# iammadab/zk

Measured on AMD Instinct MI355X. Metric: field-ops/sec (MLE fold, 2^24 evals, BN254 Fr) + sumcheck prover wall-clock, higher is better.
Workload: dtype u256 (8 x u32 Montgomery limbs, integer)

## Files before the change

zk_amd/csrc/common.cuh:

```cuda
#pragma once
#include "field.cuh"

namespace zk {

constexpr int kBlock = 256;
constexpr int kMaxFactors = 8;

struct FactorPtrs {
    const uint64_t *in[kMaxFactors];
    uint64_t *out[kMaxFactors];
};

constexpr int kMaxBatch = 8;
template <class Slot>
struct BatchOf {
    Slot a[kMaxBatch];
};
struct FactorPtrs4 {
    const uint64_t *in[4];
    uint64_t *out[4];
};
ZK_HD FactorPtrs4 factor_ptrs4(const FactorPtrs &f) {
    FactorPtrs4 r;
    for (int i = 0; i < 4; ++i) r.in[i] = f.in[i], r.out[i] = f.out[i];
// ... 95 lines not shown
struct ClaimJob {
    const uint64_t *prev_rp;
    const uint64_t *prev_chal;
    const uint64_t *w;
    uint64_t *out;
    uint32_t ns;
};
ZK_HD Fe lead_rebuild(uint32_t D, const Fe *S, const FieldParams &P) {
    const Fe L = S[D];
    if (D == 1) return fe_add(S[0], L, P);
    if (D == 2) {
        const Fe a = fe_add(S[1], L, P);
        return fe_sub(fe_add(a, a, P), S[0], P);
    }
    Fe b = fe_add(fe_sub(S[2], S[1], P), fe_add(L, L, P), P);
    b = fe_add(fe_add(b, b, P), b, P);
    return fe_add(S[0], b, P);
}

template <int CTRL>
ZK_D Fe fe_dpp(const Fe &s) {
    Fe o;
#pragma unroll
    for (int i = 0; i < 8; ++i) o.v[i] = __builtin_amdgcn_update_dpp(0u, s.v[i], CTRL, 0xF, 0xF, true);
    return o;
}
ZK_D Fe fe_wave_sum(Fe s, const FieldParams &P, uint32_t width = 64) {
    if (width > 32) {
        Fe a, b;
#pragma unroll
        for (int i = 0; i < 8; ++i) {
            const auto r = __builtin_amdgcn_permlane32_swap(s.v[i], s.v[i], false, false);
            a.v[i] = r[0];
            b.v[i] = r[1];
        }
        s = fe_add(a, b, P);
    }
    if (width > 16) {
        Fe a, b;
#pragma unroll
        for (int i = 0; i < 8; ++i) {
            const auto r = __builtin_amdgcn_permlane16_swap(s.v[i], s.v[i], false, false);
            a.v[i] = r[0];
            b.v[i] = r[1];
        }
        s = fe_add(a, b, P);
    }
    if (width > 8) s = fe_add(s, fe_dpp<0x128>(s), P);
    if (width > 4) s = fe_add(s, fe_dpp<0x12C>(s), P);
    if (width > 2) s = fe_add(s, fe_dpp<0x12E>(s), P);
    if (width > 1) s = fe_add(s, fe_dpp<0x12F>(s), P);
    return s;
}
ZK_D Fe claim_eval(const ClaimJob &cj, const FieldParams &P) {
    const uint32_t lane = threadIdx.x & 63;
    const Fe r = fe_load(cj.prev_chal, 0);
    Fe term = fe_zero();
    if (lane < cj.ns) {
        Fe one;
#pragma unroll
        for (int i = 0; i < 8; ++i) one.v[i] = P.r1[i];
        term = fe_mul(fe_load(cj.prev_rp, lane), fe_load(cj.w, lane), P);
        Fe node = fe_zero();
        for (uint32_t u = 0; u < cj.ns; ++u) {
            if (u != lane) term = fe_mul(term, fe_sub(r, node, P), P);
            node = fe_add(node, one, P);
        }
    }
    return fe_wave_sum(term, P, 8);
}

constexpr int kEvalHighMax = 12;
struct EvalHighPoint {
    uint32_t n;
    uint32_t r[kEvalHighMax][8];
};
ZK_D uint32_t eval_high_lane(uint32_t n) { return n > 8 ? 15u : n > 4 ? 7u : n > 2 ? 3u : n > 1 ? 1u : 0u; }
ZK_D Fe eval_high_weight(const EvalHighPoint &ph, uint64_t g, uint32_t lane, const FieldParams &P) {
    Fe one;
#pragma unroll
    for (int i = 0; i < 8; ++i) one.v[i] = P.r1[i];
    Fe f = one;
    for (uint32_t k = 0; k < ph.n; ++k) {
        Fe r;
#pragma unroll
        for (int i = 0; i < 8; ++i) r.v[i] = ph.r[k][i];
        const Fe sel = (g >> k) & 1 ? r : fe_sub(one, r, P);
        if ((lane & 15) == k) f = sel;
    }
    if (ph.n > 8) f = fe_mul(f, fe_dpp<0x128>(f), P);
    if (ph.n > 4) f = fe_mul(f, fe_dpp<0x124>(f), P);
    if (ph.n > 2) f = fe_mul(f, fe_dpp<0x122>(f), P);
    if (ph.n > 1) f = fe_mul(f, fe_dpp<0x121>(f), P);
    return f;
}

ZK_D Fe block_scan_excl(Fe x, Fe *red, const FieldParams &P, Fe *total) {
    const uint32_t t = threadIdx.x;
    red[t] = x;
    __syncthreads();
    for (uint32_t h = 1; h < kBlock; h <<= 1) {
        const Fe y = t >= h ? fe_mul_tt(red[t - h], red[t], P) : red[t];
        __syncthreads();
        red[t] = y;
        __syncthreads();
    }
// ... 9 lines not shown
```

zk_amd/csrc/field.cuh:

```cuda
#pragma once
#include <stdint.h>

#if defined(__HIPCC__)
#include <hip/hip_runtime.h>
#define ZK_HD __host__ __device__ __forceinline__
#define ZK_D __device__ __forceinline__
#else
#define ZK_HD inline
#define ZK_D inline
#endif

namespace zk {

struct FieldParams {
    uint32_t p[8];
    uint32_t r1[8];
    uint32_t r2[8];
    uint32_t inv;
    uint32_t bits;
    uint32_t p29[9];
    uint32_t inv29;
    uint32_t r2_29[9];
    uint32_t r2s_29[9];
};
// ... 305 lines not shown
        }
#pragma unroll
        for (int i = 0; i < 9; ++i) s[i] = borrow ? s[i] : d[i];
    }
}

struct WideAcc {
    uint32_t v[17];
};
ZK_HD void wide_zero(WideAcc &w) {
#pragma unroll
    for (int i = 0; i < 17; ++i) w.v[i] = 0;
}
template <int C>
ZK_HD void wide_mac_col(WideAcc &w, Acc &acc, const uint32_t a[8], const uint32_t b[8]) {
    constexpr int lo = C < 8 ? 0 : C - 7, hi = C < 8 ? C : 7;
    acc_add32(acc, w.v[C]);
    mac_col<hi - lo + 1>(acc, a + lo, b + (C - lo));
    w.v[C] = acc_shift(acc);
    if constexpr (C + 1 < 15) wide_mac_col<C + 1>(w, acc, a, b);
}
ZK_HD void wide_mac(WideAcc &w, const uint32_t a[8], const uint32_t b[8]) {
    Acc acc = {0, 0};
    wide_mac_col<0>(w, acc, a, b);
    acc_add32(acc, w.v[15]);
    w.v[15] = acc_shift(acc);
    w.v[16] += (uint32_t)acc.lh;
}
constexpr int kMaxLazy = 32;
ZK_HD Fe redc_wide(const WideAcc &w, const FieldParams &P) {
    uint32_t m[8];
    Acc acc = {0, 0};
    uint32_t s[9];
    redc_cols<0>(w.v, m, s, acc, P);
    s[8] = (uint32_t)acc.lh;
    {
        uint64_t c = 0;
        const uint32_t top = w.v[16];
#pragma unroll
        for (int i = 0; i < 8; ++i) {
            c += (uint64_t)top * P.r1[i] + s[i];
            s[i] = (uint32_t)c;
            c >>= 32;
        }
        s[8] += (uint32_t)c;
    }
    ladder9<4>(s, P);
    Fe r;
#pragma unroll
    for (int i = 0; i < 8; ++i) r.v[i] = s[i];
    return r;
}

ZK_HD Fe fe_reduce_u256(const uint32_t x[8], const FieldParams &P) {
    uint32_t s[9];
#pragma unroll
    for (int i = 0; i < 8; ++i) s[i] = x[i];
    s[8] = 0;
    ladder9<4>(s, P);
    Fe r;
#pragma unroll
    for (int i = 0; i < 8; ++i) r.v[i] = s[i];
    return r;
}

struct Mul29 {
    uint32_t l[9];
};
ZK_HD void split29(const uint32_t a[8], uint32_t out[9]) {
    constexpr uint32_t M = (1u << 29) - 1;
#pragma unroll
    for (int i = 0; i < 9; ++i) {
        const int bit = 29 * i, w = bit >> 5, sh = bit & 31;
        uint32_t v = a[w] >> sh;
        if (sh > 3 && w + 1 < 8) v |= a[w + 1] << (32 - sh);
        out[i] = (i < 8) ? (v & M) : v;
    }
}
ZK_HD Mul29 mul29_prepare(const Fe &c, const FieldParams &P) {
    Fe t = c;
#pragma unroll
    for (int i = 0; i < 5; ++i) t = fe_add(t, t, P);
    Mul29 m;
    split29(t.v, m.l);
    return m;
}
template <bool LAZY = false, bool TWO = false>
ZK_HD Fe mul29_core(const uint32_t (&x)[9], const uint32_t (&y)[9], const Mul29 &c, const FieldParams &P, const Mul29 *c2 = nullptr) {
    constexpr uint32_t M = (1u << 29) - 1;
    uint32_t m[9], r[9];
    uint64_t acc = 0;
#pragma unroll
    for (int k = 0; k < 9; ++k) {
#pragma unroll
        for (int i = 0; i <= k; ++i) acc += (uint64_t)x[i] * c.l[k - i];
        if constexpr (TWO) {
#pragma unroll
            for (int i = 0; i <= k; ++i) acc += (uint64_t)y[i] * c2->l[k - i];
        }
#pragma unroll
        for (int i = 0; i < k; ++i) acc += (uint64_t)m[i] * P.p29[k - i];
        m[k] = ((uint32_t)acc * P.inv29) & M;
        acc += (uint64_t)m[k] * P.p29[0];
        acc >>= 29;
    }
#pragma unroll
// ... 75 lines not shown
```

zk_amd/csrc/host_field.hpp:

```cpp
#pragma once
#include <stdint.h>
#include <string.h>

#include "field.cuh"

namespace zk {

struct FieldInfo {
    FieldParams P;
    uint32_t two_adicity;
    uint32_t generator;
    Fe two_adic_root;
    bool ready;
};

inline const uint64_t *field_modulus_limbs(int field) {
    static const uint64_t M[3][4] = {
        {0x43e1f593f0000001ULL, 0x2833e84879b97091ULL, 0xb85045b68181585dULL, 0x30644e72e131a029ULL},
        {0xffffffff00000001ULL, 0x53bda402fffe5bfeULL, 0x3339d80809a1d805ULL, 0x73eda753299d7d48ULL},
        {0x0a11800000000001ULL, 0x59aa76fed0000001ULL, 0x60b44d1e5c37b001ULL, 0x12ab655e9a2ca556ULL},
    };
    return (field >= 0 && field < 3) ? M[field] : nullptr;
}

// ... 26 lines not shown
    }
    return acc;
}
inline Fe fe_inverse(const Fe &a, const FieldParams &P) {
    uint32_t e[8], two[8] = {2, 0, 0, 0, 0, 0, 0, 0};
    sub8(e, P.p, two);
    return fe_pow_limbs(a, e, P);
}

inline const FieldInfo *field_info(int field) {
    static FieldInfo info[3];
    static const uint32_t adicity[3] = {28, 32, 47};
    static const uint32_t gen[3] = {5, 7, 22};
    if (field < 0 || field > 2) return nullptr;
    FieldInfo &I = info[field];
    if (I.ready) return &I;
    FieldParams &P = I.P;
    Fe pm = fe_from_u64limbs(field_modulus_limbs(field));
    memcpy(P.p, pm.v, 32);
    uint32_t x = 1;
    for (int i = 0; i < 5; ++i) x *= 2u - P.p[0] * x;
    P.inv = 0u - x;
    int top = 7;
    while (top > 0 && P.p[top] == 0) --top;
    P.bits = 32 * top + (32 - __builtin_clz(P.p[top]));
    uint32_t v[8] = {1, 0, 0, 0, 0, 0, 0, 0}, d[8];
    for (int i = 0; i < 512; ++i) {
        uint32_t c = add8(v, v, v);
        uint32_t b = sub8(d, v, P.p);
        if (c | (b ^ 1u)) memcpy(v, d, 32);
        if (i == 255) memcpy(P.r1, v, 32);
    }
    memcpy(P.r2, v, 32);
    split29(P.p, P.p29);
    P.inv29 = P.inv & ((1u << 29) - 1);
    {
        Fe r2;
        memcpy(r2.v, P.r2, 32);
        const Mul29 k0 = mul29_prepare(r2, P);
        Fe r2s = r2;
        for (int i = 0; i < 5; ++i) r2s = fe_add(r2s, r2s, P);
        const Mul29 k1 = mul29_prepare(r2s, P);
        memcpy(P.r2_29, k0.l, sizeof k0.l);
        memcpy(P.r2s_29, k1.l, sizeof k1.l);
    }
    {
        const int rp_log = 257 - (int)P.bits;
        int lazy_log = 0;
        while ((1 << lazy_log) < kMaxLazy) ++lazy_log;
        const int top_log = lazy_log + 2 * (int)P.bits - 512;
        const uint64_t rp = rp_log >= 0 && rp_log < 32 ? (1ull << rp_log) : ~0ull;
        const uint64_t top = top_log < 0 ? 0 : (top_log < 32 ? (1ull << top_log) : ~0ull);
        if (rp_log < 0 || rp + 1 + top >= 32 || rp + 1 + top < rp) return nullptr;
    }
    I.two_adicity = adicity[field];
    I.generator = gen[field];
    uint32_t t[8], one[8] = {1, 0, 0, 0, 0, 0, 0, 0};
    sub8(t, P.p, one);
    for (uint32_t s = 0; s < I.two_adicity; ++s) {
        for (int i = 0; i < 7; ++i) t[i] = (t[i] >> 1) | (t[i + 1] << 31);
        t[7] >>= 1;
    }
    I.two_adic_root = fe_pow_limbs(fe_from_u32(I.generator, P), t, P);
    I.ready = true;
    return &I;
}

inline bool field_root_of_unity(const FieldInfo &I, uint32_t log_n, Fe &out) {
    if (log_n > I.two_adicity) return false;
    Fe w = I.two_adic_root;
    for (uint32_t i = log_n; i < I.two_adicity; ++i) w = fe_sqr(w, I.P);
    out = w;
    return true;
}

inline void fe_to_bytes_be(const Fe &a, const FieldParams &P, uint8_t out[32]) {
    Fe c = fe_to_canonical(a, P);
    for (int i = 0; i < 8; ++i)
        for (int b = 0; b < 4; ++b) out[31 - (4 * i + b)] = (uint8_t)(c.v[i] >> (8 * b));
}
inline Fe fe_from_be_bytes_mod_order(const uint8_t *bytes, size_t len, const FieldParams &P) {
    Fe acc = fe_zero();
    const Fe c256 = fe_from_u32(256, P);
    for (size_t i = 0; i < len; ++i) acc = fe_add(fe_mul(acc, c256, P), fe_from_u32(bytes[i], P), P);
    return acc;
}

}
```

zk_amd/csrc/round_kernels.cuh:

```cuda
#pragma once
#include "common.cuh"
#include "quad.cuh"

namespace zk {

template <int NS, bool SKIP1 = false>
ZK_D void block_reduce_store(Fe (&sum)[NS], uint64_t *__restrict__ partials, const FieldParams &P) {
    __shared__ uint32_t red[kBlock / 64][NS][8];
    const int lane = threadIdx.x & 63, wave = threadIdx.x >> 6;
#pragma unroll
    for (int t = 0; t < NS; ++t) {
        if (SKIP1 && t == 1) continue;
        sum[t] = fe_wave_sum(sum[t], P);
        if (lane == 0) {
#pragma unroll
            for (int i = 0; i < 8; ++i) red[wave][t][i] = sum[t].v[i];
        }
    }
    __syncthreads();
    if (threadIdx.x < NS && !(SKIP1 && threadIdx.x == 1)) {
        const int t = threadIdx.x;
        Fe acc;
#pragma unroll
        for (int i = 0; i < 8; ++i) acc.v[i] = red[0][t][i];
        for (int w = 1; w < kBlock / 64; ++w) {
            Fe o;
#pragma unroll
            for (int i = 0; i < 8; ++i) o.v[i] = red[w][t][i];
            acc = fe_add(acc, o, P);
        }
        fe_store(partials, (uint64_t)blockIdx.x * NS + t, acc);
    }
}

template <int D, bool FUSED>
__global__ __launch_bounds__(kBlock) void k_round(FactorPtrs fp, int k, uint64_t q, FieldParams P,
                                                  const uint64_t *__restrict__ rptr, uint64_t *__restrict__ partials) {
    constexpr int NS = D + 1;
    Mul29 r = {};
    if (FUSED) r = load_challenge29(rptr);
    Fe sum[NS];
    WideAcc acc[NS];
#pragma unroll
    for (int t = 0; t < NS; ++t) {
        sum[t] = fe_zero();
        wide_zero(acc[t]);
    }
    int lazy = 0;
    const uint64_t stride = (uint64_t)gridDim.x * kBlock;
    for (uint64_t j = (uint64_t)blockIdx.x * kBlock + threadIdx.x; j < q; j += stride) {
        Fe prod[NS];
        for (int f = 0; f < k; ++f) {
            Fe lo, hi;
            if (FUSED) {
                const Fe a0 = fe_load(fp.in[f], j), a1 = fe_load(fp.in[f], j + q);
                const Fe a2 = fe_load(fp.in[f], j + 2 * q), a3 = fe_load(fp.in[f], j + 3 * q);
                lo = fe_sub(a0, fe_mul29(fe_sub(a0, a2, P), r, P), P);
                hi = fe_sub(a1, fe_mul29(fe_sub(a1, a3, P), r, P), P);
                fe_store(fp.out[f], j, lo);
                fe_store(fp.out[f], j + q, hi);
            } else {
                lo = fe_load(fp.in[f], j);
                hi = fe_load(fp.in[f], j + q);
            }
            const Fe diff = fe_sub(hi, lo, P);
            Fe v = lo;
#pragma unroll
            for (int t = 0; t < NS; ++t) {
                if (t == 1) v = hi;
                else if (t > 1) v = fe_add(v, diff, P);
                if (k == 1) sum[t] = fe_add(sum[t], v, P);
                else if (f == 0) prod[t] = v;
                else if (f < k - 1) prod[t] = fe_mul(prod[t], v, P);
                else wide_mac(acc[t], prod[t].v, v.v);
            }
        }
        if (k > 1 && ++lazy == kMaxLazy) {
#pragma unroll
            for (int t = 0; t < NS; ++t) {
                sum[t] = fe_add(sum[t], redc_wide(acc[t], P), P);
                wide_zero(acc[t]);
            }
            lazy = 0;
        }
// ... 72 lines not shown
}
#ifndef ZK_KD_MIN_BLOCKS
#define ZK_KD_MIN_BLOCKS(K, EXTRA, FUSED, SKIP1) (((K) + (EXTRA) <= 2 || ((K) == 3 && (EXTRA) == 0) || ((EXTRA) == 1 && (FUSED) && (SKIP1))) ? 2 : 1)
#endif
template <int K, int D, bool FUSED, int EXTRA = 0, bool SKIP1 = false, bool LEAD = false>
ZK_D void round_kd_body(const FactorPtrs &fp, uint64_t q, const FieldParams &P, const uint64_t *__restrict__ rptr, uint64_t *__restrict__ partials,
                        const ClaimJob &cj) {
    constexpr int NS = D + 1, NL = FUSED ? 4 : 2;
    uint32_t nblk = gridDim.x;
    if constexpr (SKIP1) {
        if (cj.out) {
            nblk -= 1;
            if (blockIdx.x == nblk) {
                if (threadIdx.x < 64) {
                    const Fe claim = claim_eval(cj, P);
                    if (threadIdx.x == 0) fe_store(cj.out, 0, claim);
                }
                return;
            }
        }
    }
    Mul29 r = {};
    if (FUSED) r = load_challenge29(rptr);
    RoundRegs<K, D, FUSED, EXTRA> R;
#pragma unroll
    for (int t = 0; t < NS; ++t) {
        R.sum[t] = fe_zero();
        if (EXTRA) R.sum_b[t] = fe_zero();
        if (K > 1) wide_zero(R.acc[t]);
    }
    const uint64_t stride = (uint64_t)nblk * kBlock;
    uint64_t j = (uint64_t)blockIdx.x * kBlock + threadIdx.x;
    if (j < q) {
#pragma unroll
        for (int f = 0; f < K + EXTRA; ++f)
#pragma unroll
            for (int l = 0; l < NL; ++l) R.cur[f][l] = fe_load(fp.in[f], j + (uint64_t)l * q);
    }
    if (RoundRegs<K, D, FUSED, EXTRA>::DEEP && j + stride < q) {
#pragma unroll
        for (int f = 0; f < K + EXTRA; ++f)
#pragma unroll
            for (int l = 0; l < NL; ++l) R.nxt[f][l] = fe_load(fp.in[f], j + stride + (uint64_t)l * q);
    }
    while (j < q) {
        const uint64_t jn = j + stride, jnn = jn + stride;
        const bool more = jn < q, more2 = jnn < q;
        round_factor<0, K, D, FUSED, EXTRA, SKIP1, LEAD>(R, fp, j, jn, more, q, r, P, jnn, more2);
        if constexpr (K + EXTRA > 1) round_factor<1, K, D, FUSED, EXTRA, SKIP1, LEAD>(R, fp, j, jn, more, q, r, P, jnn, more2);
        if constexpr (K + EXTRA > 2) round_factor<2, K, D, FUSED, EXTRA, SKIP1, LEAD>(R, fp, j, jn, more, q, r, P, jnn, more2);
        if constexpr (K + EXTRA > 3) round_factor<3, K, D, FUSED, EXTRA, SKIP1, LEAD>(R, fp, j, jn, more, q, r, P, jnn, more2);
        j = jn;
    }
    if (K > 1) {
#pragma unroll
        for (int t = 0; t < NS; ++t)
            if (!(SKIP1 && t == 1)) R.sum[t] = redc_wide(R.acc[t], P);
    }
    if (EXTRA) {
#pragma unroll
        for (int t = 0; t < NS; ++t)
            if (!(SKIP1 && t == 1)) R.sum[t] = fe_add(R.sum[t], R.sum_b[t], P);
    }
    block_reduce_store<NS, SKIP1>(R.sum, partials, P);
}
template <int K, int D, bool FUSED, int EXTRA = 0, bool SKIP1 = false, bool LEAD = false>
__global__ __launch_bounds__(kBlock, ZK_KD_MIN_BLOCKS(K, EXTRA, FUSED, SKIP1)) void k_round_kd(FactorPtrs fp, uint64_t q, FieldParams P,
                                                        const uint64_t *__restrict__ rptr, uint64_t *__restrict__ partials, ClaimJob cj = {}) {
    round_kd_body<K, D, FUSED, EXTRA, SKIP1, LEAD>(fp, q, P, rptr, partials, cj);
}
struct RoundSlot {
    FactorPtrs4 fp;
    const uint64_t *rptr;
    uint64_t *partials;
    ClaimJob cj;
};
template <int K, int D, bool FUSED, int EXTRA = 0, bool SKIP1 = false, bool LEAD = false>
__global__ __launch_bounds__(kBlock, ZK_KD_MIN_BLOCKS(K, EXTRA, FUSED, SKIP1)) void k_round_kd_b(BatchOf<RoundSlot> b, uint64_t q, FieldParams P) {
    const RoundSlot &a = b.a[blockIdx.y];
    const FactorPtrs fp = factor_ptrs_of(a.fp);
    round_kd_body<K, D, FUSED, EXTRA, SKIP1, LEAD>(fp, q, P, a.rptr, a.partials, a.cj);
}

ZK_D void dot29_mac(uint64_t (&c)[17], const uint32_t (&x)[9], const uint32_t (&y)[9]) {
#if defined(__HIP_DEVICE_COMPILE__) && !defined(ZK_NO_ASM)
    asm("v_mad_u64_u32 %0, vcc, %13, %18, %0\n\t"
        "v_mad_u64_u32 %1, vcc, %13, %19, %1\n\t"
        "v_mad_u64_u32 %2, vcc, %13, %20, %2\n\t"
        "v_mad_u64_u32 %3, vcc, %13, %21, %3\n\t"
        "v_mad_u64_u32 %4, vcc, %13, %22, %4\n\t"
        "v_mad_u64_u32 %5, vcc, %13, %23, %5\n\t"
        "v_mad_u64_u32 %6, vcc, %13, %24, %6\n\t"
        "v_mad_u64_u32 %7, vcc, %13, %25, %7\n\t"
        "v_mad_u64_u32 %8, vcc, %13, %26, %8\n\t"
        "v_mad_u64_u32 %1, vcc, %14, %18, %1\n\t"
        "v_mad_u64_u32 %2, vcc, %14, %19, %2\n\t"
        "v_mad_u64_u32 %3, vcc, %14, %20, %3\n\t"
        "v_mad_u64_u32 %4, vcc, %14, %21, %4\n\t"
        "v_mad_u64_u32 %5, vcc, %14, %22, %5\n\t"
        "v_mad_u64_u32 %6, vcc, %14, %23, %6\n\t"
        "v_mad_u64_u32 %7, vcc, %14, %24, %7\n\t"
        "v_mad_u64_u32 %8, vcc, %14, %25, %8\n\t"
        "v_mad_u64_u32 %9, vcc, %14, %26, %9\n\t"
        "v_mad_u64_u32 %2, vcc, %15, %18, %2\n\t"
        "v_mad_u64_u32 %3, vcc, %15, %19, %3\n\t"
        "v_mad_u64_u32 %4, vcc, %15, %20, %4\n\t"
        "v_mad_u64_u32 %5, vcc, %15, %21, %5\n\t"
        "v_mad_u64_u32 %6, vcc, %15, %22, %6\n\t"
        "v_mad_u64_u32 %7, vcc, %15, %23, %7\n\t"
        "v_mad_u64_u32 %8, vcc, %15, %24, %8\n\t"
        "v_mad_u64_u32 %9, vcc, %15, %25, %9\n\t"
        "v_mad_u64_u32 %10, vcc, %15, %26, %10\n\t"
        "v_mad_u64_u32 %3, vcc, %16, %18, %3\n\t"
        "v_mad_u64_u32 %4, vcc, %16, %19, %4\n\t"
        "v_mad_u64_u32 %5, vcc, %16, %20, %5\n\t"
        "v_mad_u64_u32 %6, vcc, %16, %21, %6\n\t"
        "v_mad_u64_u32 %7, vcc, %16, %22, %7\n\t"
// ... 101 lines not shown
    const uint64_t stride = (uint64_t)gridDim.x * kBlock;
    uint64_t j = (uint64_t)blockIdx.x * kBlock + threadIdx.x;
    if (j < q) {
#pragma unroll
        for (int f = 0; f < NT; ++f) cur[f][0] = fe_load(fp.in[f], j), cur[f][1] = fe_load(fp.in[f], j + q);
    }
    if (DEEP && j + stride < q) {
#pragma unroll
        for (int f = 0; f < NT; ++f) nxt[f][0] = fe_load(fp.in[f], j + stride), nxt[f][1] = fe_load(fp.in[f], j + stride + q);
    }
    int since = 0;
    while (j < q) {
        const uint64_t jn = j + stride, jnn = jn + stride;
        Fe v[NT][2];
#pragma unroll
        for (int f = 0; f < NT; ++f) v[f][0] = cur[f][0], v[f][1] = cur[f][1];
        if (DEEP) {
#pragma unroll
            for (int f = 0; f < NT; ++f) cur[f][0] = nxt[f][0], cur[f][1] = nxt[f][1];
            if (jnn < q) {
#pragma unroll
                for (int f = 0; f < NT; ++f) nxt[f][0] = fe_load(fp.in[f], jnn), nxt[f][1] = fe_load(fp.in[f], jnn + q);
            }
        } else if (jn < q) {
#pragma unroll
            for (int f = 0; f < NT; ++f) cur[f][0] = fe_load(fp.in[f], jn), cur[f][1] = fe_load(fp.in[f], jn + q);
        }
        uint32_t a[9], b[9];
        split29(v[0][0].v, a);
        split29(v[1][0].v, b);
        dot29_mac(c0, a, b);
        split29(v[0][1].v, a);
        split29(v[1][1].v, b);
        dot29_mac(c1, a, b);
        const Fe d0 = fe_sub(v[0][1], v[0][0], P), d1 = fe_sub(v[1][1], v[1][0], P);
        split29(d0.v, a);
        split29(d1.v, b);
        dot29_mac(cL, a, b);
        if (EXTRA) {
            sb0 = fe_add(sb0, v[NT - 1][0], P);
            sb1 = fe_add(sb1, v[NT - 1][1], P);
        }
        if (++since == 7) {
            dot29_normalise(c0);
            dot29_normalise(c1);
            dot29_normalise(cL);
            since = 0;
        }
        j = jn;
    }
    dot29_normalise(c0);
    dot29_normalise(c1);
    dot29_normalise(cL);
    Fe sum[3];
    {
        WideAcc w;
        dot29_to_wide(c0, w);
        sum[0] = redc_wide(w, P);
        dot29_to_wide(c1, w);
        sum[1] = redc_wide(w, P);
        dot29_to_wide(cL, w);
        sum[2] = redc_wide(w, P);
    }
    if (EXTRA) {
        sum[0] = fe_add(sum[0], sb0, P);
        sum[1] = fe_add(sum[1], sb1, P);
    }
    block_reduce_store<3>(sum, partials, P);
}
template <int EXTRA>
__global__ __launch_bounds__(kBlock, 2) void k_round0_dot29(FactorPtrs fp, uint64_t q, FieldParams P, uint64_t *__restrict__ partials) {
    round0_dot29_body<EXTRA>(fp, q, P, partials);
}
template <int EXTRA>
__global__ __launch_bounds__(kBlock, 2) void k_round0_dot29_b(BatchOf<RoundSlot> b, uint64_t q, FieldParams P) {
    const RoundSlot &a = b.a[blockIdx.y];
    const FactorPtrs fp = factor_ptrs_of(a.fp);
    round0_dot29_body<EXTRA>(fp, q, P, a.partials);
}

extern __shared__ __attribute__((aligned(1024))) uint8_t glds_ring[];
constexpr uint32_t kGldsRingBytes = 4 * 8192, kGldsRing3Bytes = 4 * 12288;
template <int N>
ZK_D void wait_vm() {
    asm volatile("s_waitcnt vmcnt(%0)" ::"n"(N) : "memory");
}
#define ZK_GLDS_PIECES(ADDR)                      \
    "global_load_lds_dwordx4 %1, " ADDR " nt\n\t" \
    "global_load_lds_dwordx4 %1, " ADDR " offset:1024 nt\n\t"
#define ZK_GLDS_ROW(M0, ADDR) "s_mov_b32 m0, " M0 "\n\ts_nop 0\n\t" ZK_GLDS_PIECES(ADDR)
ZK_D void glds_rows2(uint64_t a0, uint64_t a1, uint32_t voff, uint32_t lds_dst) {
    unsigned keep;
    asm volatile("s_mov_b32 %0, m0\n\t" ZK_GLDS_ROW("%4", "%2") ZK_GLDS_ROW("%5", "%3") "s_mov_b32 m0, %0"
                 : "=&s"(keep)
                 : "v"(voff), "s"(a0), "s"(a1), "s"(lds_dst), "s"(lds_dst + 2048u)
                 : "memory");
}
ZK_D void glds_rows4(uint64_t a0, uint64_t a1, uint64_t a2, uint64_t a3, uint32_t voff, uint32_t lds_dst) {
    unsigned keep;
    asm volatile("s_mov_b32 %0, m0\n\t" ZK_GLDS_ROW("%6", "%2") ZK_GLDS_ROW("%7", "%3") ZK_GLDS_ROW("%8", "%4") ZK_GLDS_ROW("%9", "%5") "s_mov_b32 m0, %0"
                 : "=&s"(keep)
                 : "v"(voff), "s"(a0), "s"(a1), "s"(a2), "s"(a3), "s"(lds_dst), "s"(lds_dst + 2048u), "s"(lds_dst + 4096u), "s"(lds_dst + 6144u)
                 : "memory");
}
#undef ZK_GLDS_ROW
#undef ZK_GLDS_PIECES
ZK_D Fe glds_elem(const uint8_t *row, uint32_t elem) {
    const uint4 *p = reinterpret_cast<const uint4 *>(row + elem * 32);
    const uint4 a = p[0], b = p[1];
    Fe r = {{a.x, a.y, a.z, a.w, b.x, b.y, b.z, b.w}};
    return r;
}
struct GldsWave {
    uint8_t *my;
    uint32_t my_lds;
    uint32_t lane, voff, own;
    uint64_t r0, rs, K;
};
ZK_D GldsWave glds_wave(uint64_t q, uint32_t nblk, uint32_t bytes_per_wave = 8192) {
    GldsWave w;
    w.lane = threadIdx.x & 63;
// ... 116 lines not shown
    if (F + 1 < NT) {
        const uint64_t a = (uint64_t)(uintptr_t)fp.in[F + 1 < NT ? F + 1 : 0] + run * 2048;
        glds_rows4(a, a + rowb, a + 2 * rowb, a + 3 * rowb, w.voff, w.my_lds);
    } else if (!last) {
        const uint64_t a = (uint64_t)(uintptr_t)fp.in[0] + (run + w.rs) * 2048;
        glds_rows4(a, a + rowb, a + 2 * rowb, a + 3 * rowb, w.voff, w.my_lds);
    }
    const Fe lo = fe_sub(c0, fe_mul29(fe_sub(c0, c2, P), r, P), P);
    const Fe hi = fe_sub(c1, fe_mul29(fe_sub(c1, c3, P), r, P), P);
    uint64_t *out = fp.out[F];
    if (STORE_NT) {
        run_store_nt(out + run * 256, w.lane, lo);
        run_store_nt(out + (run * 64 + q) * 4, w.lane, hi);
    } else {
        run_store(out + run * 256, w.lane, lo);
        run_store(out + (run * 64 + q) * 4, w.lane, hi);
    }
    const Fe diff = fe_sub(hi, lo, P);
    Fe v = lo;
#pragma unroll
    for (int t = 0; t <= D; ++t) {
        if (t == 1) {
            v = hi;
            continue;
        }
        if (t == D) v = diff;
        else if (t > 1) v = fe_add(v, diff, P);
        if (F == K) {
            if (t < D) sum_b[t] = fe_add(sum_b[t], v, P);
        } else if (F == 0) prod[t] = v;
        else if (F < K - 1) prod[t] = ZK_KD_INNER_MUL(prod[t], v, P);
        else wide_mac(acc[t], prod[t].v, v.v);
    }
    if (F + 1 < NT || !last) wait_vm<4>();
}
template <int K, int EXTRA, bool STORE_NT>
ZK_D void fused_glds_body(const FactorPtrs &fp, uint64_t q, const FieldParams &P, const uint64_t *__restrict__ rptr, uint64_t *__restrict__ partials,
                          const ClaimJob &cj) {
    constexpr int NS = K + 1;
    uint32_t nblk = gridDim.x;
    if (cj.out) {
        nblk -= 1;
        if (blockIdx.x == nblk) {
            if (threadIdx.x < 64) {
                const Fe claim = claim_eval(cj, P);
                if (threadIdx.x == 0) fe_store(cj.out, 0, claim);
            }
            return;
        }
    }
    const Mul29 r = load_challenge29(rptr);
    asm volatile("s_waitcnt vmcnt(0)" ::: "memory");
    const GldsWave w = glds_wave(q, nblk);
    Fe prod[NS], sum[NS], sum_b[NS];
    WideAcc acc[NS];
#pragma unroll
    for (int t = 0; t < NS; ++t) {
        sum[t] = fe_zero();
        sum_b[t] = fe_zero();
        wide_zero(acc[t]);
    }
    if (w.K) {
        {
            const uint64_t a = (uint64_t)(uintptr_t)fp.in[0] + w.r0 * 2048, rowb = q * 32;
            glds_rows4(a, a + rowb, a + 2 * rowb, a + 3 * rowb, w.voff, w.my_lds);
        }
        wait_vm<0>();
        for (uint64_t k = 0; k < w.K; ++k) {
            const uint64_t run = w.r0 + k * w.rs;
            const bool last = k + 1 == w.K;
            fused_glds_unit<0, K, EXTRA, STORE_NT>(w, fp, q, run, last, r, P, prod, acc, sum_b);
            fused_glds_unit<1, K, EXTRA, STORE_NT>(w, fp, q, run, last, r, P, prod, acc, sum_b);
            if constexpr (K + EXTRA > 2) fused_glds_unit<2, K, EXTRA, STORE_NT>(w, fp, q, run, last, r, P, prod, acc, sum_b);
            if constexpr (K + EXTRA > 3) fused_glds_unit<3, K, EXTRA, STORE_NT>(w, fp, q, run, last, r, P, prod, acc, sum_b);
        }
#pragma unroll
        for (int t = 0; t < NS; ++t)
            if (t != 1) sum[t] = redc_wide(acc[t], P);
        if (EXTRA) {
#pragma unroll
            for (int t = 0; t < K; ++t)
                if (t != 1) sum[t] = fe_add(sum[t], sum_b[t], P);
        }
    }
    block_reduce_store<NS, true>(sum, partials, P);
}
template <int K, int EXTRA, bool STORE_NT>
__global__ __launch_bounds__(kBlock, 2) void k_round_fused_glds(FactorPtrs fp, uint64_t q, FieldParams P, const uint64_t *__restrict__ rptr,
                                                                 uint64_t *__restrict__ partials, ClaimJob cj) {
    fused_glds_body<K, EXTRA, STORE_NT>(fp, q, P, rptr, partials, cj);
}
template <int K, int EXTRA, bool STORE_NT>
__global__ __launch_bounds__(kBlock, 2) void k_round_fused_glds_b(BatchOf<RoundSlot> b, uint64_t q, FieldParams P) {
    const RoundSlot &a = b.a[blockIdx.y];
    const FactorPtrs fp = factor_ptrs_of(a.fp);
    fused_glds_body<K, EXTRA, STORE_NT>(fp, q, P, a.rptr, a.partials, a.cj);
}

template <int K, int D, int EXTRA>
ZK_D void round_quad_body(const FactorPtrs &fp, uint64_t q, const FieldParams &P, const uint64_t *__restrict__ rptr, uint64_t *__restrict__ partials) {
    constexpr int NF = K + EXTRA, NS = D + 1;
    static_assert(NF <= 4 && NS <= 4, "four lanes per pair index");
    __shared__ uint32_t red[kBlock / 64][4][8];
    const Mul29 r = load_challenge29(rptr);
    const uint32_t lane = threadIdx.x & 63, wave = threadIdx.x >> 6, l4 = lane & 3;
    const bool has_factor = l4 < (uint32_t)NF;
    const uint64_t *in = fp.in[0];
    uint64_t *out = fp.out[0];
#pragma unroll
    for (int f = 1; f < NF; ++f)
        if (l4 == (uint32_t)f) {
            in = fp.in[f];
            out = fp.out[f];
        }
    const uint64_t stride = (uint64_t)gridDim.x * (kBlock / 4);
    uint64_t j = (uint64_t)blockIdx.x * (kBlock / 4) + (threadIdx.x >> 2);
    WideAcc acc;
    wide_zero(acc);
    Fe sum = fe_zero();
    Fe cur[4];
#pragma unroll
    for (int l = 0; l < 4; ++l) cur[l] = fe_zero();
    if (j < q && has_factor) {
#pragma unroll
        for (int l = 0; l < 4; ++l) cur[l] = fe_load(in, j + (uint64_t)l * q);
    }
    while (j < q) {
        const uint64_t jn = j + stride;
        Fe v[NS];
        v[0] = fe_sub(cur[0], fe_mul29(fe_sub(cur[0], cur[2], P), r, P), P);
        const Fe hi = fe_sub(cur[1], fe_mul29(fe_sub(cur[1], cur[3], P), r, P), P);
        if (has_factor) {
            fe_store(out, j, v[0]);
            fe_store(out, j + q, hi);
            if (jn < q) {
#pragma unroll
                for (int l = 0; l < 4; ++l) cur[l] = fe_load(in, jn + (uint64_t)l * q);
            }
        }
        if constexpr (NS > 1) v[1] = hi;
        if constexpr (NS > 2) {
            const Fe diff = fe_sub(hi, v[0], P);
#pragma unroll
            for (int t = 2; t < NS; ++t) v[t] = fe_add(v[t - 1], diff, P);
        }
        Fe w[NF];
#pragma unroll
        for (int g = 0; g < NF; ++g) w[g] = fe_zero();
        quad_transpose<0, NF, NS>(v, w, l4);
        if constexpr (K == 1) {
            sum = fe_add(sum, w[0], P);
        } else {
            Fe prod = w[0];
#pragma unroll
            for (int g = 1; g + 1 < K; ++g) prod = ZK_KD_INNER_MUL(prod, w[g], P);
            wide_mac(acc, prod.v, w[K - 1].v);
        }
        if constexpr (EXTRA) sum = fe_add(sum, w[K], P);
        j = jn;
    }
    Fe s = sum;
    if constexpr (K > 1) s = fe_add(redc_wide(acc, P), sum, P);
    {
        Fe a, b;
#pragma unroll
        for (int i = 0; i < 8; ++i) {
            const auto x = __builtin_amdgcn_permlane32_swap(s.v[i], s.v[i], false, false);
            a.v[i] = x[0];
            b.v[i] = x[1];
        }
        s = fe_add(a, b, P);
#pragma unroll
        for (int i = 0; i < 8; ++i) {
            const auto x = __builtin_amdgcn_permlane16_swap(s.v[i], s.v[i], false, false);
            a.v[i] = x[0];
            b.v[i] = x[1];
        }
        s = fe_add(a, b, P);
        s = fe_add(s, fe_dpp<0x128>(s), P);
        s = fe_add(s, fe_dpp<0x12C>(s), P);
    }
    if (lane < 4) {
#pragma unroll
        for (int i = 0; i < 8; ++i) red[wave][lane][i] = s.v[i];
    }
    __syncthreads();
    if (threadIdx.x < (uint32_t)NS) {
        Fe tot = fe_zero();
        for (int wv = 0; wv < kBlock / 64; ++wv) {
            Fe o;
#pragma unroll
            for (int i = 0; i < 8; ++i) o.v[i] = red[wv][threadIdx.x][i];
            tot = fe_add(tot, o, P);
        }
        fe_store(partials, (uint64_t)blockIdx.x * NS + threadIdx.x, tot);
    }
}
template <int K, int D, int EXTRA>
__global__ __launch_bounds__(kBlock) void k_round_quad(FactorPtrs fp, uint64_t q, FieldParams P, const uint64_t *__restrict__ rptr,
                                                       uint64_t *__restrict__ partials) {
    round_quad_body<K, D, EXTRA>(fp, q, P, rptr, partials);
}
template <int K, int D, int EXTRA>
__global__ __launch_bounds__(kBlock) void k_round_quad_b(BatchOf<RoundSlot> b, uint64_t q, FieldParams P) {
    const RoundSlot &a = b.a[blockIdx.y];
    const FactorPtrs fp = factor_ptrs_of(a.fp);
    round_quad_body<K, D, EXTRA>(fp, q, P, a.rptr, a.partials);
}

__global__ __launch_bounds__(kBlock) void k_round_single_t(FactorPtrs fp, int k, uint64_t q, FieldParams P, Fe tval,
                                                           uint64_t *__restrict__ partials) {
    Fe sum[1] = {fe_zero()};
    const uint64_t stride = (uint64_t)gridDim.x * kBlock;
    for (uint64_t j = (uint64_t)blockIdx.x * kBlock + threadIdx.x; j < q; j += stride) {
        Fe prod = fe_zero();
        for (int f = 0; f < k; ++f) {
            const Fe lo = fe_load(fp.in[f], j), hi = fe_load(fp.in[f], j + q);
            const Fe v = fe_sub(lo, fe_mul(tval, fe_sub(lo, hi, P), P), P);
            prod = (f == 0) ? v : fe_mul(prod, v, P);
        }
        sum[0] = fe_add(sum[0], prod, P);
    }
    block_reduce_store<1>(sum, partials, P);
}

}
```

Before: 195.2 billion.

## Defer Montgomery reduction of wide accumulators to block level

Instead of each thread reducing its 17-limb wide accumulator with redc_wide before the block reduction, the unreduced wide accumulators are summed across the wave with permlane swaps and inline DPP add-with-carry asm, then across waves in shared memory. A single block-level redc with a quotient-estimate correction finishes the job. This removes per-thread Montgomery reductions in the round kernels, in exchange for reducing 17 words instead of 8 per lane and adding a host-side bound check that may reject fields whose headroom is insufficient.

```diff
diff --git a/zk_amd/csrc/common.cuh b/zk_amd/csrc/common.cuh
--- a/zk_amd/csrc/common.cuh
+++ b/zk_amd/csrc/common.cuh
@@ -171,6 +171,81 @@
     if (width > 1) s = fe_add(s, fe_dpp<0x12F>(s), P);
     return s;
 }
+template <int CTRL>
+ZK_D WideAcc wide_dpp(const WideAcc &s) {
+    WideAcc o;
+#pragma unroll
+    for (int i = 0; i < 17; ++i) o.v[i] = __builtin_amdgcn_update_dpp(0u, s.v[i], CTRL, 0xF, 0xF, true);
+    return o;
+}
+#define ZK_WIDE_ROR(N)                                                                                         \
+    "s_nop 1\n\t"                                                                                              \
+    "v_add_co_u32_dpp %0, vcc, %0, %0 row_ror:" #N " row_mask:0xf bank_mask:0xf\n\t"                           \
+    "v_addc_co_u32_dpp %1, vcc, %1, %1, vcc row_ror:" #N " row_mask:0xf bank_mask:0xf\n\t"                     \
+    "v_addc_co_u32_dpp %2, vcc, %2, %2, vcc row_ror:" #N " row_mask:0xf bank_mask:0xf\n\t"                     \
+    "v_addc_co_u32_dpp %3, vcc, %3, %3, vcc row_ror:" #N " row_mask:0xf bank_mask:0xf\n\t"                     \
+    "v_addc_co_u32_dpp %4, vcc, %4, %4, vcc row_ror:" #N " row_mask:0xf bank_mask:0xf\n\t"                     \
+    "v_addc_co_u32_dpp %5, vcc, %5, %5, vcc row_ror:" #N " row_mask:0xf bank_mask:0xf\n\t"                     \
+    "v_addc_co_u32_dpp %6, vcc, %6, %6, vcc row_ror:" #N " row_mask:0xf bank_mask:0xf\n\t"                     \
+    "v_addc_co_u32_dpp %7, vcc, %7, %7, vcc row_ror:" #N " row_mask:0xf bank_mask:0xf\n\t"                     \
+    "v_addc_co_u32_dpp %8, vcc, %8, %8, vcc row_ror:" #N " row_mask:0xf bank_mask:0xf\n\t"                     \
+    "v_addc_co_u32_dpp %9, vcc, %9, %9, vcc row_ror:" #N " row_mask:0xf bank_mask:0xf\n\t"                     \
+    "v_addc_co_u32_dpp %10, vcc, %10, %10, vcc row_ror:" #N " row_mask:0xf bank_mask:0xf\n\t"                  \
+    "v_addc_co_u32_dpp %11, vcc, %11, %11, vcc row_ror:" #N " row_mask:0xf bank_mask:0xf\n\t"                  \
+    "v_addc_co_u32_dpp %12, vcc, %12, %12, vcc row_ror:" #N " row_mask:0xf bank_mask:0xf\n\t"                  \
+    "v_addc_co_u32_dpp %13, vcc, %13, %13, vcc row_ror:" #N " row_mask:0xf bank_mask:0xf\n\t"                  \
+    "v_addc_co_u32_dpp %14, vcc, %14, %14, vcc row_ror:" #N " row_mask:0xf bank_mask:0xf\n\t"                  \
+    "v_addc_co_u32_dpp %15, vcc, %15, %15, vcc row_ror:" #N " row_mask:0xf bank_mask:0xf\n\t"                  \
+    "v_addc_co_u32_dpp %16, vcc, %16, %16, vcc row_ror:" #N " row_mask:0xf bank_mask:0xf"
+template <int N>
+ZK_D void wide_add_row_ror(WideAcc &s) {
+    static_assert(N == 8 || N == 4 || N == 2 || N == 1, "the four levels inside a row");
+#if defined(__HIP_DEVICE_COMPILE__) && !defined(ZK_NO_ASM)
+#define ZK_WIDE_OPS                                                                                                                         \
+    "+v"(s.v[0]), "+v"(s.v[1]), "+v"(s.v[2]), "+v"(s.v[3]), "+v"(s.v[4]), "+v"(s.v[5]), "+v"(s.v[6]), "+v"(s.v[7]), "+v"(s.v[8]), "+v"(s.v[9]), \
+        "+v"(s.v[10]), "+v"(s.v[11]), "+v"(s.v[12]), "+v"(s.v[13]), "+v"(s.v[14]), "+v"(s.v[15]), "+v"(s.v[16])
+    if constexpr (N == 8) asm(ZK_WIDE_ROR(8) : ZK_WIDE_OPS : : "vcc");
+    else if constexpr (N == 4) asm(ZK_WIDE_ROR(4) : ZK_WIDE_OPS : : "vcc");
+    else if constexpr (N == 2) asm(ZK_WIDE_ROR(2) : ZK_WIDE_OPS : : "vcc");
+    else asm(ZK_WIDE_ROR(1) : ZK_WIDE_OPS : : "vcc");
+#undef ZK_WIDE_OPS
+#else
+    wide_add(s, wide_dpp<0x120 + N>(s));
+#endif
+}
+#undef ZK_WIDE_ROR
+template <bool QUAD = false>
+ZK_D WideAcc wide_wave_sum(WideAcc s) {
+    {
+        WideAcc a, b;
+#pragma unroll
+        for (int i = 0; i < 17; ++i) {
+            const auto r = __builtin_amdgcn_permlane32_swap(s.v[i], s.v[i], false, false);
+            a.v[i] = r[0];
+            b.v[i] = r[1];
+        }
+        wide_add(a, b);
+        s = a;
+    }
+    {
+        WideAcc a, b;
+#pragma unroll
+        for (int i = 0; i < 17; ++i) {
+            const auto r = __builtin_amdgcn_permlane16_swap(s.v[i], s.v[i], false, false);
+            a.v[i] = r[0];
+            b.v[i] = r[1];
+        }
+        wide_add(a, b);
+        s = a;
+    }
+    wide_add_row_ror<8>(s);
+    wide_add_row_ror<4>(s);
+    if constexpr (!QUAD) {
+        wide_add_row_ror<2>(s);
+        wide_add_row_ror<1>(s);
+    }
+    return s;
+}
 ZK_D Fe claim_eval(const ClaimJob &cj, const FieldParams &P) {
     const uint32_t lane = threadIdx.x & 63;
     const Fe r = fe_load(cj.prev_chal, 0);
diff --git a/zk_amd/csrc/field.cuh b/zk_amd/csrc/field.cuh
--- a/zk_amd/csrc/field.cuh
+++ b/zk_amd/csrc/field.cuh
@@ -381,6 +381,54 @@
     return r;
 }
 
+ZK_HD void wide_add(WideAcc &a, const WideAcc &b) {
+    uint32_t c = 0;
+#pragma unroll
+    for (int i = 0; i < 17; ++i) {
+        uint32_t co;
+        a.v[i] = __builtin_addc(a.v[i], b.v[i], c, &co);
+        c = co;
+    }
+}
+constexpr int kBlockLazyLog = 13;
+ZK_HD Fe redc_wide_block(const WideAcc &w, const FieldParams &P) {
+    uint32_t m[8];
+    Acc acc = {0, 0};
+    uint32_t s[9];
+    redc_cols<0>(w.v, m, s, acc, P);
+    s[8] = (uint32_t)acc.lh;
+    {
+        uint64_t c = 0;
+        const uint32_t top = w.v[16];
+#pragma unroll
+        for (int i = 0; i < 8; ++i) {
+            c += (uint64_t)top * P.r1[i] + s[i];
+            s[i] = (uint32_t)c;
+            c >>= 32;
+        }
+        s[8] += (uint32_t)c;
+    }
+    {
+        const uint32_t a = (s[7] >> 18) | (s[8] << 14), b = (P.p[7] >> 18) + 1;
+        const uint32_t qh = a / b;
+        uint64_t c = 0;
+        uint32_t borrow = 0;
+#pragma unroll
+        for (int i = 0; i < 9; ++i) {
+            if (i < 8) c += (uint64_t)qh * P.p[i];
+            uint32_t bo;
+            s[i] = __builtin_subc(s[i], (uint32_t)c, borrow, &bo);
+            borrow = bo;
+            c >>= 32;
+        }
+    }
+    ladder9<1>(s, P);
+    Fe r;
+#pragma unroll
+    for (int i = 0; i < 8; ++i) r.v[i] = s[i];
+    return r;
+}
+
 ZK_HD Fe fe_reduce_u256(const uint32_t x[8], const FieldParams &P) {
     uint32_t s[9];
 #pragma unroll
diff --git a/zk_amd/csrc/host_field.hpp b/zk_amd/csrc/host_field.hpp
--- a/zk_amd/csrc/host_field.hpp
+++ b/zk_amd/csrc/host_field.hpp
@@ -102,6 +102,11 @@
         const uint64_t rp = rp_log >= 0 && rp_log < 32 ? (1ull << rp_log) : ~0ull;
         const uint64_t top = top_log < 0 ? 0 : (top_log < 32 ? (1ull << top_log) : ~0ull);
         if (rp_log < 0 || rp + 1 + top >= 32 || rp + 1 + top < rp) return nullptr;
+        uint32_t pp[16];
+        mul_wide(pp, P.p, P.p);
+        const uint64_t top_block = pp[15] >> (32 - kBlockLazyLog);
+        const uint64_t q_max = rp + 1 + top_block;
+        if (q_max >= (1u << 11) || q_max + 1 >= (uint64_t)(P.p[7] >> 18) + 1) return nullptr;
     }
     I.two_adicity = adicity[field];
     I.generator = gen[field];
diff --git a/zk_amd/csrc/round_kernels.cuh b/zk_amd/csrc/round_kernels.cuh
--- a/zk_amd/csrc/round_kernels.cuh
+++ b/zk_amd/csrc/round_kernels.cuh
@@ -30,6 +30,53 @@
             acc = fe_add(acc, o, P);
         }
         fe_store(partials, (uint64_t)blockIdx.x * NS + t, acc);
+    }
+}
+
+template <int NS, bool SKIP1 = false, int NB = 0>
+ZK_D void block_reduce_store_wide(WideAcc (&acc)[NS], const Fe *sum_b, uint64_t *__restrict__ partials, const FieldParams &P) {
+    static_assert(NB <= NS, "one extra sum per slot at most");
+    __shared__ uint32_t redw[kBlock / 64][NS][17];
+    __shared__ uint32_t redb[kBlock / 64][NB ? NB : 1][8];
+    const int lane = threadIdx.x & 63, wave = threadIdx.x >> 6;
+#pragma unroll
+    for (int t = 0; t < NS; ++t) {
+        if (SKIP1 && t == 1) continue;
+        const WideAcc s = wide_wave_sum(acc[t]);
+        if (lane == 0) {
+#pragma unroll
+            for (int i = 0; i < 17; ++i) redw[wave][t][i] = s.v[i];
+        }
+        if (t < NB) {
+            const Fe b = fe_wave_sum(sum_b[t], P);
+            if (lane == 0) {
+#pragma unroll
+                for (int i = 0; i < 8; ++i) redb[wave][t][i] = b.v[i];
+            }
+        }
+    }
+    __syncthreads();
+    if (threadIdx.x < NS && !(SKIP1 && threadIdx.x == 1)) {
+        const int t = threadIdx.x;
+        WideAcc w;
+#pragma unroll
+        for (int i = 0; i < 17; ++i) w.v[i] = redw[0][t][i];
+        for (int wv = 1; wv < kBlock / 64; ++wv) {
+            WideAcc o;
+#pragma unroll
+            for (int i = 0; i < 17; ++i) o.v[i] = redw[wv][t][i];
+            wide_add(w, o);
+        }
+        Fe r = redc_wide_block(w, P);
+        if (t < NB) {
+            for (int wv = 0; wv < kBlock / 64; ++wv) {
+                Fe o;
+#pragma unroll
+                for (int i = 0; i < 8; ++i) o.v[i] = redb[wv][t][i];
+                r = fe_add(r, o, P);
+            }
+        }
+        fe_store(partials, (uint64_t)blockIdx.x * NS + t, r);
     }
 }
 
@@ -208,17 +255,16 @@
         if constexpr (K + EXTRA > 3) round_factor<3, K, D, FUSED, EXTRA, SKIP1, LEAD>(R, fp, j, jn, more, q, r, P, jnn, more2);
         j = jn;
     }
-    if (K > 1) {
-#pragma unroll
-        for (int t = 0; t < NS; ++t)
-            if (!(SKIP1 && t == 1)) R.sum[t] = redc_wide(R.acc[t], P);
-    }
-    if (EXTRA) {
-#pragma unroll
-        for (int t = 0; t < NS; ++t)
-            if (!(SKIP1 && t == 1)) R.sum[t] = fe_add(R.sum[t], R.sum_b[t], P);
-    }
-    block_reduce_store<NS, SKIP1>(R.sum, partials, P);
+    if constexpr (K > 1) {
+        block_reduce_store_wide<NS, SKIP1, EXTRA ? (LEAD ? D : NS) : 0>(R.acc, R.sum_b, partials, P);
+    } else {
+        if (EXTRA) {
+#pragma unroll
+            for (int t = 0; t < NS; ++t)
+                if (!(SKIP1 && t == 1)) R.sum[t] = fe_add(R.sum[t], R.sum_b[t], P);
+        }
+        block_reduce_store<NS, SKIP1>(R.sum, partials, P);
+    }
 }
 template <int K, int D, bool FUSED, int EXTRA = 0, bool SKIP1 = false, bool LEAD = false>
 __global__ __launch_bounds__(kBlock, ZK_KD_MIN_BLOCKS(K, EXTRA, FUSED, SKIP1)) void k_round_kd(FactorPtrs fp, uint64_t q, FieldParams P,
@@ -426,21 +472,12 @@
     dot29_normalise(c0);
     dot29_normalise(c1);
     dot29_normalise(cL);
-    Fe sum[3];
-    {
-        WideAcc w;
-        dot29_to_wide(c0, w);
-        sum[0] = redc_wide(w, P);
-        dot29_to_wide(c1, w);
-        sum[1] = redc_wide(w, P);
-        dot29_to_wide(cL, w);
-        sum[2] = redc_wide(w, P);
-    }
-    if (EXTRA) {
-        sum[0] = fe_add(sum[0], sb0, P);
-        sum[1] = fe_add(sum[1], sb1, P);
-    }
-    block_reduce_store<3>(sum, partials, P);
+    WideAcc w[3];
+    dot29_to_wide(c0, w[0]);
+    dot29_to_wide(c1, w[1]);
+    dot29_to_wide(cL, w[2]);
+    const Fe sb[2] = {sb0, sb1};
+    block_reduce_store_wide<3, false, EXTRA ? 2 : 0>(w, sb, partials, P);
 }
 template <int EXTRA>
 __global__ __launch_bounds__(kBlock, 2) void k_round0_dot29(FactorPtrs fp, uint64_t q, FieldParams P, uint64_t *__restrict__ partials) {
@@ -663,11 +700,10 @@
     const Mul29 r = load_challenge29(rptr);
     asm volatile("s_waitcnt vmcnt(0)" ::: "memory");
     const GldsWave w = glds_wave(q, nblk);
-    Fe prod[NS], sum[NS], sum_b[NS];
+    Fe prod[NS], sum_b[NS];
     WideAcc acc[NS];
 #pragma unroll
     for (int t = 0; t < NS; ++t) {
-        sum[t] = fe_zero();
         sum_b[t] = fe_zero();
         wide_zero(acc[t]);
     }
@@ -685,16 +721,8 @@
             if constexpr (K + EXTRA > 2) fused_glds_unit<2, K, EXTRA, STORE_NT>(w, fp, q, run, last, r, P, prod, acc, sum_b);
             if constexpr (K + EXTRA > 3) fused_glds_unit<3, K, EXTRA, STORE_NT>(w, fp, q, run, last, r, P, prod, acc, sum_b);
         }
-#pragma unroll
-        for (int t = 0; t < NS; ++t)
-            if (t != 1) sum[t] = redc_wide(acc[t], P);
-        if (EXTRA) {
-#pragma unroll
-            for (int t = 0; t < K; ++t)
-                if (t != 1) sum[t] = fe_add(sum[t], sum_b[t], P);
-        }
-    }
-    block_reduce_store<NS, true>(sum, partials, P);
+    }
+    block_reduce_store_wide<NS, true, EXTRA ? K : 0>(acc, sum_b, partials, P);
 }
 template <int K, int EXTRA, bool STORE_NT>
 __global__ __launch_bounds__(kBlock, 2) void k_round_fused_glds(FactorPtrs fp, uint64_t q, FieldParams P, const uint64_t *__restrict__ rptr,
@@ -770,9 +798,16 @@
         if constexpr (EXTRA) sum = fe_add(sum, w[K], P);
         j = jn;
     }
+    __shared__ uint32_t redw[K > 1 ? kBlock / 64 : 1][4][17];
+    if constexpr (K > 1) {
+        const WideAcc sw = wide_wave_sum<true>(acc);
+        if (lane < 4) {
+#pragma unroll
+            for (int i = 0; i < 17; ++i) redw[wave][lane][i] = sw.v[i];
+        }
+    }
     Fe s = sum;
-    if constexpr (K > 1) s = fe_add(redc_wide(acc, P), sum, P);
-    {
+    if constexpr (K == 1 || EXTRA != 0) {
         Fe a, b;
 #pragma unroll
         for (int i = 0; i < 8; ++i) {
@@ -798,7 +833,19 @@
     __syncthreads();
     if (threadIdx.x < (uint32_t)NS) {
         Fe tot = fe_zero();
-        for (int wv = 0; wv < kBlock / 64; ++wv) {
+        if constexpr (K > 1) {
+            WideAcc w;
+#pragma unroll
+            for (int i = 0; i < 17; ++i) w.v[i] = redw[0][threadIdx.x][i];
+            for (int wv = 1; wv < kBlock / 64; ++wv) {
+                WideAcc o;
+#pragma unroll
+                for (int i = 0; i < 17; ++i) o.v[i] = redw[wv][threadIdx.x][i];
+                wide_add(w, o);
+            }
+            tot = redc_wide_block(w, P);
+        }
+        for (int wv = 0; wv < (K == 1 || EXTRA != 0 ? kBlock / 64 : 0); ++wv) {
             Fe o;
 #pragma unroll
             for (int i = 0; i < 8; ++i) o.v[i] = red[wv][threadIdx.x][i];
```

Result: no change. 196.9 billion (median of 3 runs) (+0.9%).
